# microsoft/UniSpeech

Hardware: AMD Instinct MI355X
Metric: audio-seconds/sec pretraining, WavLM-Base 15s@16kHz (higher is better)
Workload: dtype bf16; 1 GPU; WavLM-Base (12L, d=768) pretrain fwd+bwd+grad-reduce+fused-Adam, bf16, batch=32x15s per GPU, masked-pred loss (BASELINE.json configs[1]); global_batch=32, frames_per_utt=749, parallelism=dp1, optimizer=fused Adam, fp32 master, clip 10

## Files before the change

### include/wavlm_hip.h

```cpp
#ifndef WAVLM_HIP_H
#define WAVLM_HIP_H
#include <stddef.h>
#include <stdint.h>
#ifdef __cplusplus
extern "C" {
#endif

#define WAVLM_HIP_ABI_VERSION 29
int wavlm_abi_version(void);

typedef struct wavlm_gemm_desc {
  int32_t dtype;
  int32_t c_dtype;
  int32_t M, N, K, KB;
  int32_t transA, transB;
  int64_t lda, ldb, ldc;
  int64_t sA_kb, sB_kb;
  int32_t batch_o, batch_i;
  int64_t sA_o, sA_i, sB_o, sB_i, sC_o, sC_i;
  const void* A;
  const void* B;
  void* C;
  float alpha;
  int32_t epi;
// ... 208 lines not shown
  void* y;
  void* r_out;
  void* saved; uint64_t saved_bytes;
  void* workspace; uint64_t ws_bytes;
  const void* dy;
  const void* dr_out;
  void* dx;
  void* dr_in;
  float* dtab;
} wavlm_layer_desc;
uint64_t wavlm_layer_saved_bytes(const wavlm_layer_desc* d);
uint64_t wavlm_layer_fwd_workspace_bytes(const wavlm_layer_desc* d);
uint64_t wavlm_layer_bwd_workspace_bytes(const wavlm_layer_desc* d);
int wavlm_encoder_layer_fwd(const wavlm_layer_desc* d, void* stream);
int wavlm_encoder_layer_bwd(const wavlm_layer_desc* d, void* stream);

typedef void (*wavlm_grad_listener)(const void* base, uint64_t bytes, void* stream, void* user);
void wavlm_dp_set_listener(wavlm_grad_listener cb, void* user);

int wavlm_dp_unique_id(void* id128);
int wavlm_dp_init(int32_t rank, int32_t world, const void* id128, int32_t average);
int wavlm_dp_bucket_ready(void* base, uint64_t count, int32_t dtype, void* compute_stream);
int wavlm_dp_finish(void* compute_stream);
int wavlm_dp_destroy(void);

uint64_t wavlm_kmeans_centres_bytes(int32_t K, int32_t D);
int wavlm_kmeans_prepare(const float* C, int32_t K, int32_t D, void* image, uint64_t image_bytes, void* stream);
int wavlm_kmeans_assign(const void* X, int32_t x_dtype, int64_t N, int32_t D, int64_t ldx, const void* image, int32_t K,
                        int32_t* labels, float* min_dist, void* stream);
uint64_t wavlm_kmeans_accumulate_workspace_bytes(int64_t N, int32_t K, int32_t D);
// ... 72 lines not shown
```

### unispeech_amd/_lib.py

```python
import ctypes as C
import os

_HERE = os.path.dirname(os.path.abspath(__file__))
LIB_PATH = os.environ.get("WAVLM_HIP_LIB") or os.path.join(_HERE, "lib", "libwavlm_hip.so")

_lib = None
ABI_VERSION = 29

F32, BF16, I16 = 0, 1, 2

c_i32, c_i64, c_u64, c_f32, c_vp = C.c_int32, C.c_int64, C.c_uint64, C.c_float, C.c_void_p


class ConvRelayoutDesc(C.Structure):
    _fields_ = [("W", c_vp * 8), ("Wf", c_vp * 8), ("Wb", c_vp * 8),
                ("Cout", c_i32 * 8), ("Cin", c_i32 * 8), ("k", c_i32 * 8), ("s", c_i32 * 8),
                ("n_layers", c_i32), ("dtype", c_i32)]


class GemmDesc(C.Structure):
    _fields_ = [
        ("dtype", c_i32), ("c_dtype", c_i32),
        ("M", c_i32), ("N", c_i32), ("K", c_i32), ("KB", c_i32),
        ("transA", c_i32), ("transB", c_i32),
# ... 174 lines not shown
    "wavlm_mfcc_rows": (c_i32, [c_vp, c_i32, c_i64, c_i32, c_i64, c_vp, c_i32, c_i32, c_i32, c_vp, c_vp, c_vp, c_vp, c_i32, c_vp,
                                c_vp, c_i64, c_i64, c_i32, c_vp]),
    "wavlm_fbank_supported": (c_i32, [c_i32, c_i32, c_i32, c_i32]),
    "wavlm_fbank_frames": (c_i64, [c_i64, c_i32, c_i32]),
    "wavlm_fbank_rows": (c_i32, [c_vp, c_i32, c_i64, c_i32, c_i64, c_vp, c_i32, c_i32, c_i32, c_i32, c_vp, c_vp, c_vp, c_vp, c_i32,
                                 c_vp, c_i64, c_i64, c_vp]),
    "wavlm_dp_set_listener": (None, [c_vp, c_vp]),
    "wavlm_dp_unique_id": (c_i32, [c_vp]),
    "wavlm_dp_init": (c_i32, [c_i32, c_i32, c_vp, c_i32]),
    "wavlm_dp_bucket_ready": (c_i32, [c_vp, c_u64, c_i32, c_vp]),
    "wavlm_dp_finish": (c_i32, [c_vp]),
    "wavlm_dp_destroy": (c_i32, []),
    "wavlm_prof_enable": (None, [c_i32]),
    "wavlm_gemm_set_variant": (None, [c_i32]),
    "wavlm_set_reserved_cus": (None, [c_i32]),
    "wavlm_get_reserved_cus": (c_i32, []),
    "wavlm_prof_collect": (c_i32, [c_i32, C.POINTER(C.c_double), C.POINTER(C.c_double)]),
    "wavlm_prof_collect_bytes": (C.c_double, [c_i32]),
    "wavlm_prof_collect_class": (c_i32, [c_i32, C.POINTER(C.c_double), C.POINTER(C.c_double), C.POINTER(C.c_double)]),
    "wavlm_prof_dump": (c_i32, [C.c_char_p]),
}

_ERR = {-1: "invalid argument", -2: "kernel launch failure", -3: "out of memory"}


class WavlmHipError(RuntimeError):
    pass


def lib():
# ... 22 lines not shown
```

### unispeech_amd/csrc/attn_fused.hip

```cpp
#include "attn_fused.hpp"

typedef float f32x2_t __attribute__((ext_vector_type(2)));
#if !defined(WAVLM_EXPERIMENTAL)
#undef FA_FWD_LAZY
#undef FA_FWD_THETA
#undef FA_DQ_PK
#endif
#ifndef FA_FWD_LAZY
#define FA_FWD_LAZY 0
#endif
#ifndef FA_FWD_THETA
#define FA_FWD_THETA 8.f
#endif
#ifndef FA_DQ_PK
#define FA_DQ_PK 1
#endif
#if !defined(WAVLM_EXPERIMENTAL)
#undef FA_FWD_MFMA_SUM
#endif
#ifndef FA_FWD_MFMA_SUM
#define FA_FWD_MFMA_SUM 0
#endif
#ifndef FA_FWD_BIAS_IN_C
#define FA_FWD_BIAS_IN_C 1
// ... 780 lines not shown
    for (int f2 = 0; f2 < 2; ++f2)
#pragma unroll
      for (int q4 = 0; q4 < 4; ++q4) {
        uint2 w;
        w.x = pack_bf16(dq[f2][4 * q4] * p.scale, dq[f2][4 * q4 + 1] * p.scale);
        w.y = pack_bf16(dq[f2][4 * q4 + 2] * p.scale, dq[f2][4 * q4 + 3] * p.scale);
        *reinterpret_cast<uint2*>(dst + 32 * f2 + 8 * q4 + 4 * hi) = w;
      }
    if (hi == 0) {
      p.delta[(long)bh * T + i] = dl;
      if (p.dgate) p.dgate[(long)bh * T + i] = dg;
    }
  }
}

__global__ __launch_bounds__(1024) void fa_dtab_reduce_kernel(const float* __restrict__ part, float* __restrict__ out,
                                                              int B, int H, int nqt, int L, int Lp, int T, int nkv, int accumulate) {
  __shared__ float4 red[64][17];
  const int col = threadIdx.x & 15, slice = threadIdx.x >> 4;
  const int d = (blockIdx.x * 16 + col) * 4;
  const int h = blockIdx.y;
  const int nrow = nqt * 4, ntot = B * nrow, span = 64 * nkv + 32;
  float4 acc[4];
#pragma unroll
  for (int u = 0; u < 4; ++u) acc[u] = make_float4(0.f, 0.f, 0.f, 0.f);
  if (d < Lp) {
    for (int r0 = slice; r0 < ntot; r0 += 256) {
#pragma unroll
      for (int u = 0; u < 4; ++u) {
        const int r = r0 + 64 * u;
        if (r < ntot) {
          const int b = r / nrow, c = r - b * nrow;
          const int k0 = d - (T - 1 - 32 * c - 31);
          if (k0 > -4 && k0 < span) {
            const float4 v = *reinterpret_cast<const float4*>(part + (((long)b * H + h) * nrow + c) * Lp + d);
            acc[u].x += (k0 >= 0 && k0 < span) ? v.x : 0.f;
            acc[u].y += (k0 + 1 >= 0 && k0 + 1 < span) ? v.y : 0.f;
            acc[u].z += (k0 + 2 >= 0 && k0 + 2 < span) ? v.z : 0.f;
            acc[u].w += (k0 + 3 >= 0 && k0 + 3 < span) ? v.w : 0.f;
          }
        }
      }
    }
  }
  float4 t;
  t.x = (acc[0].x + acc[1].x) + (acc[2].x + acc[3].x); t.y = (acc[0].y + acc[1].y) + (acc[2].y + acc[3].y);
  t.z = (acc[0].z + acc[1].z) + (acc[2].z + acc[3].z); t.w = (acc[0].w + acc[1].w) + (acc[2].w + acc[3].w);
  red[slice][col] = t;
  __syncthreads();
  if (slice < 4) {
    float4 q = make_float4(0.f, 0.f, 0.f, 0.f);
#pragma unroll
    for (int k = 0; k < 16; ++k) { const float4 v = red[slice * 16 + k][col]; q.x += v.x; q.y += v.y; q.z += v.z; q.w += v.w; }
    red[slice * 16][col] = q;
  }
  __syncthreads();
  if (slice == 0 && d < L) {
    const float4 a0 = red[0][col], a1 = red[16][col], a2 = red[32][col], a3 = red[48][col];
    const float o[4] = {(a0.x + a1.x) + (a2.x + a3.x), (a0.y + a1.y) + (a2.y + a3.y), (a0.z + a1.z) + (a2.z + a3.z),
                        (a0.w + a1.w) + (a2.w + a3.w)};
#pragma unroll
    for (int k = 0; k < 4; ++k)
      if (d + k < L) out[(long)h * L + d + k] = accumulate ? out[(long)h * L + d + k] + o[k] : o[k];
  }
}

static FaP fa_params(int B, int H, int T, float scale, float p_drop, uint64_t seed) {
  FaP p;
  p.B = B; p.H = H; p.T = T; p.scale = scale;
  p.sc2 = scale * FA_LOG2E;
  double tt = (double)p_drop * 65536.0 + 0.5; if (tt > 65535.0) tt = 65535.0;
  p.th = p_drop > 0.f ? (unsigned)tt : 0u;
  if (p_drop > 0.f && p.th == 0u) p.th = 1u;
  p.sc = p.th ? (float)(1.0 / (1.0 - (double)p.th / 65536.0)) : 1.f;
  p.log2sc = log2f(p.sc); p.inv_sc = 1.f / p.sc;
  p.ths = (int)p.th - 32768;
  p.k2 = (unsigned)((p.ths - 1) & 0xffff) * 0x10001u;
  p.k3 = (unsigned)(p.ths & 0xffff) * 0x10001u;
  p.ps.P16 = nullptr; p.ps.mt = nullptr;
// ... 158 lines not shown
  if (use64) {
    p.nqb = (T + FA_K64 - 1) / FA_K64;
    const int rc = fa_launch_dkv64(p, (unsigned)(p.nqb * B * H), st);
    if (rc != WL_OK) return rc;
  } else {
    p.nqb = (T + FA_BK1 - 1) / FA_BK1;
    const dim3 grid2((unsigned)(p.nqb * B * H));
    const int rc = fa_launch_dkv(p, grid2.x, smem2, st);
    if (rc != WL_OK) return rc;
  }
  if (dbias) {
    const int rcb = wl_colsum_finish(p.dbias_part, B * nqt * 4, 3 * H * FA_HD, dbias, dbias_dtype, dbias_accumulate, st);
    if (rcb != WL_OK) return rcb;
    if (dbias_accumulate && !wl_fin_active()) wl_notify_grad(dbias, (uint64_t)3 * H * FA_HD * wl_esize(dbias_dtype), stream);
  }
  if (tab)
    WL_LAUNCH(fa_dtab_reduce_kernel, dim3((unsigned)((Lp / 4 + 15) / 16), (unsigned)H), dim3(1024), 0, st,
              (const float*)p.dtab_part, dtab, (int)B, (int)H, nqt, L, Lp, (int)T, (T + FA_BKV - 1) / FA_BKV, (int)dtab_accumulate);
  return wl_check_launch();
}
```

### unispeech_amd/csrc/common.hpp

```cpp
#pragma once
#include <hip/hip_runtime.h>
#include <stdint.h>
#include <stdio.h>
#include <mutex>

#define WL_MAX_DEVICES 64

#define WL_OK 0
#define WL_EINVAL (-1)
#define WL_ELAUNCH (-2)
#define WL_ENOMEM (-3)

enum { WL_F32 = 0, WL_BF16 = 1, WL_I16 = 2 };

typedef unsigned short bf16_t;

__device__ __forceinline__ float bf2f(bf16_t v) {
  return __uint_as_float(((unsigned)v) << 16);
}
__device__ __forceinline__ bf16_t f2bf(float f) {
  const __bf16 h = (__bf16)f;
  return __builtin_bit_cast(bf16_t, h);
}
__device__ __forceinline__ unsigned pack_bf16x2(float a, float b) {
// ... 157 lines not shown
  wl_launch_failed = 0;
  return e ? WL_ELAUNCH : WL_OK;
}

void wl_notify_grad(const void* base, uint64_t bytes, void* stream);
static inline uint64_t wl_esize(int dt) { return dt == WL_BF16 ? 2 : 4; }
int wl_attn_fused_bwd_ex(const void* qkv, const void* O, const void* dO, const float* lse, const float* gate,
                         const float* tab, const uint8_t* kpm, const void* pstore, uint64_t pstore_bytes, void* dqkv, float* dgate,
                         float* dtab, int dtab_accumulate,
                         void* dbias, int32_t dbias_dtype, int32_t dbias_accumulate, int32_t B, int32_t H, int32_t T,
                         int32_t head_dim, float scale, float p_drop, uint64_t seed, void* workspace, uint64_t ws_bytes,
                         void* stream);
int wl_colsum_finish(const float* part, int nblk, int n, void* out, int out_dtype, int accumulate, hipStream_t st);

struct WlFinSeg { const float* part; void* out; long stride, rep_stride; int nblk, n, out_dtype, accumulate, rep, blk0; };
#define WL_FIN_MAX 16
struct WlFinList { WlFinSeg s[WL_FIN_MAX]; int n, blocks; };
void wl_fin_defer(WlFinList* l);
bool wl_fin_active();
bool wl_fin_add(const float* part, int nblk, long stride, int n, void* out, int out_dtype, int accumulate, int rep = 1,
                long rep_stride = 0);
int wl_fin_flush(WlFinList& l, void* stream);
```

### unispeech_amd/csrc/gemm_bf16.hip

```cpp
#include <atomic>

#include "gemm_common.hpp"
#include "split_policy.hpp"

#include "tile_loaders.hpp"

template <bool TA, bool TB, int BM, int BN, int WM, int WN, bool VEC>
__global__ __launch_bounds__(WM * WN * 64) void gemm_bf16_kernel(GemmP p) {
  constexpr int FM = BM / WM / 32, FN = BN / WN / 32;
  constexpr int NT = WM * WN * 64;
  static_assert((WM * WN == 4 || WM * WN == 8) && FM >= 1 && FN >= 1, "4 or 8 waves");
  constexpr int A_BYTES = BM * 128, B_BYTES = BN * 128;
  extern __shared__ __attribute__((aligned(16))) unsigned char smem[];

  int tile;
  {
    const int nt = p.tiles_m * p.tiles_n, bid = blockIdx.x;
    const int q = nt >> 3, rem = nt & 7, xcd = bid & 7, idx = bid >> 3;
    tile = (xcd < rem ? xcd * (q + 1) : rem * (q + 1) + (xcd - rem) * q) + idx;
  }
  const int tn = tile % p.tiles_n, tm = tile / p.tiles_n;
  const int z = blockIdx.y, split = blockIdx.z;
  const int zo = z / p.batch_i, zi = z % p.batch_i;
  const int m0 = tm * BM, n0 = tn * BN;
// ... 151 lines not shown
      for (int u = 0; u < 4; ++u) {
        v[0] += a[u].x; v[1] += a[u].y; v[2] += a[u].z; v[3] += a[u].w;
        v[4] += b[u].x; v[5] += b[u].y; v[6] += b[u].z; v[7] += b[u].w;
      }
    }
    for (; k < S; ++k) {
      const float4 a = *reinterpret_cast<const float4*>(src + (long)k * mn);
      const float4 b = *reinterpret_cast<const float4*>(src + (long)k * mn + 4);
      v[0] += a.x; v[1] += a.y; v[2] += a.z; v[3] += a.w; v[4] += b.x; v[5] += b.y; v[6] += b.z; v[7] += b.w;
    }
    const int m = (int)(r / p.N), n = (int)(r - (long)m * p.N);
    gemm_store8(q, z / p.batch_i, z % p.batch_i, z, 0, m, n, v);
  }
}

struct RedGrpP {
  float* ws[4]; void* C[4]; long ldc[4]; int M[4], N[4], c_dtype[4], accumulate[4]; float alpha[4];
  long base[5]; int n, S;
};
__global__ __launch_bounds__(256) void gemm_splitk_reduce8_grouped_kernel(RedGrpP p) {
  const long total8 = p.base[p.n];
  for (long i8 = (long)blockIdx.x * blockDim.x + threadIdx.x; i8 < total8; i8 += (long)gridDim.x * blockDim.x) {
    const int g = (i8 >= p.base[1]) + (i8 >= p.base[2]) + (i8 >= p.base[3]);
    const long i = (i8 - p.base[g]) << 3;
    const int N = p.N[g];
    const long mn = (long)p.M[g] * N;
    const float* src = p.ws[g] + i;
    float v[8];
#pragma unroll
    for (int e = 0; e < 8; ++e) v[e] = 0.f;
    for (int k = 0; k < p.S; ++k) {
      const float4 a = *reinterpret_cast<const float4*>(src + (long)k * mn);
      const float4 b = *reinterpret_cast<const float4*>(src + (long)k * mn + 4);
      v[0] += a.x; v[1] += a.y; v[2] += a.z; v[3] += a.w; v[4] += b.x; v[5] += b.y; v[6] += b.z; v[7] += b.w;
    }
    const long m = i / N, n = i - m * N;
    const long off = m * p.ldc[g] + n;
#pragma unroll
    for (int e = 0; e < 8; ++e) v[e] *= p.alpha[g];
    if (p.accumulate[g]) {
      float c[8];
      ld8_dt(p.C[g], off, p.c_dtype[g], c);
#pragma unroll
      for (int e = 0; e < 8; ++e) v[e] += c[e];
    }
    st8_dt(p.C[g], off, p.c_dtype[g], v);
  }
}

template <bool TA, bool TB, int BM, int BN, int WM, int WN>
static int launch_cfg(GemmP& p, int nbatch, bool vec, hipStream_t st) {
  p.tiles_m = (p.M + BM - 1) / BM;
  p.tiles_n = (p.N + BN - 1) / BN;
  dim3 grid((unsigned)(p.tiles_m * p.tiles_n), (unsigned)nbatch, (unsigned)p.split_k);
  constexpr size_t smem = 2 * (size_t)(BM + BN) * 128;
  constexpr int nt = WM * WN * 64;
  if (smem > 65536) {
    static bool done_v = false, done_s = false;
    bool& done = vec ? done_v : done_s;
    if (!done) {
      const void* fn = vec ? (const void*)gemm_bf16_kernel<TA, TB, BM, BN, WM, WN, true>
                           : (const void*)gemm_bf16_kernel<TA, TB, BM, BN, WM, WN, false>;
// ... 355 lines not shown
    static const bool spread = [] { const char* e = getenv("WAVLM_SK_SPREAD"); return !(e && *e == '0'); }();
    p.sk_spread = spread && (plan.s * tiles_all) % 8 == 0 && plan.R % 8 == 0 && G % 8 == 0;
  }
  const int pi = prof_begin(d, st);
  if (pi >= 0) {
    g_prof.flops[pi] = flops;
    double by = 0.0;
    for (int i = 0; i < n; ++i) by += 2.0 * ((double)d[i].M * d[i].K + (double)d[i].N * d[i].K) + 2.0 * 2.0 * d[i].M * d[i].N;
    g_prof.bytes[pi] = by;
    int* sh = g_prof.shape[pi];
    sh[0] = -n; sh[1] = 0; sh[2] = d->K; sh[3] = 1; sh[4] = 3; sh[5] = 0; sh[6] = sk ? 0 : p.split_k; sh[7] = n;
  }
  const bool fixup = w4_takes(d, true) && gemm_w4_fixup_ok(p);
  p.fix_epoch = fixup ? 1u : 0u; p.fix_cnt = nullptr; p.fix_flag = nullptr;
  int rc = w4_takes(d, true) ? gemm_w4_launch_grouped(p, st) : gemm_pp_launch_grouped(p, st);
  if (rc == WL_OK && !fixup) {
    RedGrpP r;
    r.n = n; r.S = p.split_k; r.base[0] = 0;
    for (int i = 0; i < 4; ++i) {
      const wavlm_gemm_desc* e = d + (i < n ? i : n - 1);
      r.ws[i] = (float*)e->workspace; r.C[i] = e->C; r.ldc[i] = e->ldc; r.M[i] = e->M; r.N[i] = e->N;
      r.c_dtype[i] = e->c_dtype; r.accumulate[i] = e->accumulate; r.alpha[i] = e->alpha;
      r.base[i + 1] = i < n ? r.base[i] + (((long)e->M * e->N) >> 3) : 0x7fffffffffffffffL;
    }
    const long total8 = r.base[n];
    long blocks = (total8 + 255) / 256; if (blocks > 4096) blocks = 4096;
    WL_LAUNCH(gemm_splitk_reduce8_grouped_kernel, dim3((unsigned)blocks), dim3(256), 0, st, r);
    rc = wl_check_launch();
  }
  prof_end(pi, st);
  if (rc == WL_OK)
    for (int i = 0; i < n; ++i) gemm_notify(d + i, false, stream);
  return rc;
}
```

### unispeech_amd/csrc/layer.hip

```cpp
#include <stdlib.h>
#include <string.h>

#include <atomic>

#include "common.hpp"
#include "split_policy.hpp"
#include "wavlm_hip.h"

static std::atomic<wavlm_grad_listener> g_listener{nullptr};
static std::atomic<void*> g_listener_user{nullptr};
void wl_notify_grad(const void* base, uint64_t bytes, void* stream) {
  const wavlm_grad_listener cb = g_listener.load(std::memory_order_acquire);
  if (cb && base && bytes) cb(base, bytes, stream, g_listener_user.load(std::memory_order_acquire));
}
extern "C" void wavlm_dp_set_listener(wavlm_grad_listener cb, void* user) {
  g_listener.store(nullptr, std::memory_order_release);
  g_listener_user.store(user, std::memory_order_release);
  g_listener.store(cb, std::memory_order_release);
}

namespace {

inline uint64_t rup256(uint64_t v) { return (v + 255) & ~(uint64_t)255; }

// ... 114 lines not shown
  w.da = d->p_drop > 0.f ? c.take(n * D * 2) : w.dxa;
  w.dO = c.take(n * D * 2);
  w.dqkv = c.take(n * 3 * D * 2);
  if (d->tab) w.dgate = (float*)c.take((uint64_t)d->B * d->H * d->T * 4);
  w.ln_b = wavlm_layernorm_bwd_workspace_bytes(d->D); w.ln_ws = c.take(w.ln_b); w.ln_ws2 = c.take(w.ln_b);
  w.cs_b = lin_dx_colsum_ws((int64_t)n, d->F);
  if (w.cs_b < wavlm_colsum_workspace_bytes(d->D)) w.cs_b = wavlm_colsum_workspace_bytes(d->D);
  w.cs_ws = c.take(w.cs_b); w.cs_ws2 = c.take(w.cs_b);
  w.attn_b = wavlm_attn_fused_bwd_workspace_bytes(d->B, d->H, d->T); w.attn_ws = c.take(w.attn_b);
  w.gate_b = wavlm_gate_bwd_workspace_bytes(d->H, 64); w.gate_ws = c.take(w.gate_b);
  const wavlm_wgrad_item it[4] = {{nullptr, nullptr, nullptr, d->D, d->F}, {nullptr, nullptr, nullptr, d->F, d->D},
                                  {nullptr, nullptr, nullptr, d->D, d->D}, {nullptr, nullptr, nullptr, 3 * d->D, d->D}};
  w.wg_b = wavlm_linear_wgrads_workspace_bytes(it, 4, (int64_t)n); w.wg_ws = c.take(w.wg_b);
  w.bytes = c.off;
  if (base && !c.ok) w.bytes = ~(uint64_t)0;
  return w;
}

}

#if defined(WAVLM_EXPERIMENTAL)
extern "C" int wavlm_lab_build(void) { return 1; }
#endif

extern "C" {

static long grid_or(int32_t grid) { return grid > 0 ? grid : wl_policy::grid_blocks(); }
static int forced_or(int32_t forced) { return forced >= 0 ? forced : wl_policy::forced_split(); }
int32_t wavlm_grid_blocks(void) { return wl_policy::grid_blocks(); }
int32_t wavlm_wgrad_grouping(void) { return wl_policy::grouping() ? 1 : 0; }
// ... 15 lines not shown
    const long t = wg_tiles(it[i]);
    int s = wl_policy::split_single(it[i].N, it[i].K, kt, G);
    const int gs = wl_policy::slabs_grouped(t, kt, G, forced, false);
    if (gs > s) s = gs;
    if (balanced && t < G && G / t + 1 > s) s = (int)(G / t) + 1;
    tot += rup256((uint64_t)s * it[i].N * it[i].K * 4);
  }
  return tot;
}

int wavlm_linear_wgrads(const wavlm_wgrad_item* it, int32_t cnt, int64_t n, int32_t pdt, void* ws, uint64_t wsb, void* stream) {
  if (!it || cnt <= 0 || n <= 0 || (pdt != WL_BF16 && pdt != WL_F32)) return WL_EINVAL;
  for (int i = 0; i < cnt; ++i)
    if (!it[i].dy || !it[i].x || !it[i].dW || it[i].N <= 0 || it[i].K <= 0) return WL_EINVAL;
  const long kt = (long)((n + 63) / 64);
  int i = 0;
  while (i < cnt) {
    int j = i; long tiles = 0;
    while (wl_policy::grouping() && j < cnt && j - i < 4) {
      const long t = wg_tiles(it[j]);
      if (j > i && wavlm_split_grouped(tiles + t, kt, 0, -1) < 2) break;
      tiles += t; ++j;
    }
    if (j == i) j = i + 1;
    const int m = j - i;
    Carver c(ws, wsb);
    if (m >= 2) {
      const int split = wavlm_slabs_grouped(tiles, kt, 0, -1, -1);
      wavlm_gemm_desc g[4];
      for (int k = 0; k < m; ++k) {
        wg_desc(g[k], it[i + k], n, pdt, split);
        g[k].ws_bytes = wavlm_gemm_workspace_bytes(&g[k]);
        g[k].workspace = c.take(g[k].ws_bytes);
      }
      if (!c.ok) return WL_EINVAL;
      const int rc = wavlm_gemm_grouped(g, m, stream);
      if (rc != WL_OK) return rc;
    } else {
      wavlm_gemm_desc g;
      wg_desc(g, it[i], n, pdt, wavlm_split_single(it[i].N, it[i].K, kt, 0));
      if (g.split_k > 1) { g.ws_bytes = wavlm_gemm_workspace_bytes(&g); g.workspace = c.take(g.ws_bytes); if (!c.ok) return WL_EINVAL; }
// ... 139 lines not shown
```

### unispeech_amd/csrc/rowops.hip

```cpp
#include "common.hpp"
#include <stdlib.h>
#include "../../include/wavlm_hip.h"

__device__ __forceinline__ void load8(const float* p, float (&v)[8]) {
  const float4 a = *reinterpret_cast<const float4*>(p);
  const float4 b = *reinterpret_cast<const float4*>(p + 4);
  v[0] = a.x; v[1] = a.y; v[2] = a.z; v[3] = a.w; v[4] = b.x; v[5] = b.y; v[6] = b.z; v[7] = b.w;
}
__device__ __forceinline__ void load8(const bf16_t* p, float (&v)[8]) {
  const uint4 a = *reinterpret_cast<const uint4*>(p);
  v[0] = __uint_as_float(a.x << 16); v[1] = __uint_as_float(a.x & 0xffff0000u);
  v[2] = __uint_as_float(a.y << 16); v[3] = __uint_as_float(a.y & 0xffff0000u);
  v[4] = __uint_as_float(a.z << 16); v[5] = __uint_as_float(a.z & 0xffff0000u);
  v[6] = __uint_as_float(a.w << 16); v[7] = __uint_as_float(a.w & 0xffff0000u);
}
__device__ __forceinline__ void store8(float* p, const float (&v)[8]) {
  *reinterpret_cast<float4*>(p) = make_float4(v[0], v[1], v[2], v[3]);
  *reinterpret_cast<float4*>(p + 4) = make_float4(v[4], v[5], v[6], v[7]);
}
__device__ __forceinline__ void store8(bf16_t* p, const float (&v)[8]) {
  uint4 o;
  o.x = pack_bf16x2(v[0], v[1]); o.y = pack_bf16x2(v[2], v[3]);
  o.z = pack_bf16x2(v[4], v[5]); o.w = pack_bf16x2(v[6], v[7]);
  *reinterpret_cast<uint4*>(p) = o;
// ... 486 lines not shown
    }
    __syncthreads();
    for (int i = threadIdx.x; i < 64 * VEC; i += 256) {
      const int col = c * 64 * VEC + i;
      pg[col] = red[0][0][i] + red[1][0][i] + red[2][0][i] + red[3][0][i];
      pg[D + col] = red[0][1][i] + red[1][1][i] + red[2][1][i] + red[3][1][i];
      if constexpr (CS) pg[2 * D + col] = red[0][2][i] + red[1][2][i] + red[2][2][i] + red[3][2][i];
    }
  }
}

__global__ __launch_bounds__(1024) void colsum_finish_kernel(const float* __restrict__ part, int nblk, long stride, int n,
                                                              void* out, int out_dtype, int accumulate, long part_y, void* out_y,
                                                              void* out_z) {
  __shared__ float red[64][17];
  const int col = threadIdx.x & 15, slice = threadIdx.x >> 4;
  const int c = blockIdx.x * 16 + col;
  if (blockIdx.y) { part += part_y * blockIdx.y; out = blockIdx.y == 1 ? out_y : out_z; }
  float s = 0.f;
  if (c < n) {
    float s0 = 0.f, s1 = 0.f, s2 = 0.f, s3 = 0.f;
    int b = slice;
    for (; b + 192 < nblk; b += 256) {
      s0 += part[(long)b * stride + c];
      s1 += part[(long)(b + 64) * stride + c];
      s2 += part[(long)(b + 128) * stride + c];
      s3 += part[(long)(b + 192) * stride + c];
    }
    for (; b < nblk; b += 64) s0 += part[(long)b * stride + c];
    s = (s0 + s1) + (s2 + s3);
  }
  red[slice][col] = s;
  __syncthreads();
  if (slice < 4) {
    float t = 0.f;
#pragma unroll
    for (int k = 0; k < 16; ++k) t += red[slice * 16 + k][col];
    red[slice * 16][col] = t;
  }
  __syncthreads();
  if (slice == 0 && c < n) {
    s = (red[0][col] + red[16][col]) + (red[32][col] + red[48][col]);
    if (accumulate) s += ld_elem(out, c, out_dtype);
    st_elem(out, c, out_dtype, s);
  }
}

__global__ __launch_bounds__(1024) void colsum_finish_multi_kernel(WlFinList L) {
  __shared__ float red[64][17];
  int si = 0;
#pragma unroll 1
  for (int k = 1; k < L.n; ++k) if ((int)blockIdx.x >= L.s[k].blk0) si = k;
  const WlFinSeg& g = L.s[si];
  const float* __restrict__ part = g.part;
  const long stride = g.stride;
  const int nblk = g.nblk, n = g.n;
  const int col = threadIdx.x & 15, slice = threadIdx.x >> 4;
  const int c = ((int)blockIdx.x - g.blk0) * 16 + col;
  float s = 0.f;
  if (c < n) {
    float s0 = 0.f, s1 = 0.f, s2 = 0.f, s3 = 0.f;
    int b = slice;
    for (; b + 192 < nblk; b += 256) {
      s0 += part[(long)b * stride + c];
      s1 += part[(long)(b + 64) * stride + c];
      s2 += part[(long)(b + 128) * stride + c];
      s3 += part[(long)(b + 192) * stride + c];
    }
    for (; b < nblk; b += 64) s0 += part[(long)b * stride + c];
    s = (s0 + s1) + (s2 + s3);
  }
  red[slice][col] = s;
  __syncthreads();
  if (slice < 4) {
    float t = 0.f;
#pragma unroll
    for (int k = 0; k < 16; ++k) t += red[slice * 16 + k][col];
    red[slice * 16][col] = t;
  }
  __syncthreads();
  if (slice == 0 && c < n) {
    s = (red[0][col] + red[16][col]) + (red[32][col] + red[48][col]);
    for (int r = 0; r < g.rep; ++r) {
      const long idx = (long)r * g.rep_stride + c;
      st_elem(g.out, idx, g.out_dtype, g.accumulate ? s + ld_elem(g.out, idx, g.out_dtype) : s);
    }
  }
}

static thread_local WlFinList* g_fin_list = nullptr;
void wl_fin_defer(WlFinList* l) { g_fin_list = l; if (l) { l->n = 0; l->blocks = 0; } }
bool wl_fin_active() { return g_fin_list != nullptr; }
bool wl_fin_add(const float* part, int nblk, long stride, int n, void* out, int out_dtype, int accumulate, int rep, long rep_stride) {
  WlFinList* l = g_fin_list;
  if (!l || l->n >= WL_FIN_MAX || n <= 0) return false;
  WlFinSeg& g = l->s[l->n++];
  g.part = part; g.out = out; g.stride = stride; g.rep_stride = rep_stride; g.nblk = nblk; g.n = n; g.out_dtype = out_dtype;
  g.accumulate = accumulate; g.rep = rep < 1 ? 1 : rep; g.blk0 = l->blocks;
  l->blocks += (n + 15) / 16;
  return true;
}
int wl_fin_flush(WlFinList& l, void* stream) {
  if (l.n == 0) return WL_OK;
  WL_LAUNCH(colsum_finish_multi_kernel, dim3((unsigned)l.blocks), dim3(1024), 0, (hipStream_t)stream, l);
  const int rc = wl_check_launch();
  if (rc == WL_OK)
    for (int k = 0; k < l.n; ++k) {
      const WlFinSeg& g = l.s[k];
      if (g.accumulate) wl_notify_grad(g.out, (uint64_t)((long)(g.rep - 1) * g.rep_stride + g.n) * wl_esize(g.out_dtype), stream);
    }
  l.n = 0; l.blocks = 0;
  return rc;
}

#define CS_MAXC 8
template <typename T>
__global__ __launch_bounds__(256) void colsum_partial_kernel(const T* __restrict__ x, long rows, int N, long ld,
    const unsigned char* __restrict__ inc, const unsigned char* __restrict__ exc, float* __restrict__ part) {
  __shared__ float red[4][512];
  const int lane = threadIdx.x & 63, wave = threadIdx.x >> 6;
  const int nch = N >> 3;
  float acc[CS_MAXC][8];
#pragma unroll
  for (int c = 0; c < CS_MAXC; ++c)
#pragma unroll
    for (int e = 0; e < 8; ++e) acc[c][e] = 0.f;
// ... 531 lines not shown
```

Measured before the change: 14590 audio-s/s.

## Merge split-K slab, relative-bias and colsum finish reductions into one deferred kernel

Split-K grouped weight-gradient reductions and the attention relative-position-bias gradient reduction can now be deferred into the existing finish list and run in a single merged kernel alongside the bias column-sum finishes. The goal is fewer small kernel launches and less serialization at the end of each layer's backward pass. To make deferral safe, the weight-grad workspace carver stops reusing its buffer across groups while merging, and workspace overlap checks are added. This costs more workspace, delays gradient notifications until the flush, and uses a larger block size for the slab reduction.

```diff
diff --git a/include/wavlm_hip.h b/include/wavlm_hip.h
--- a/include/wavlm_hip.h
+++ b/include/wavlm_hip.h
@@ -6,7 +6,7 @@
 extern "C" {
 #endif
 
-#define WAVLM_HIP_ABI_VERSION 29
+#define WAVLM_HIP_ABI_VERSION 30
 int wavlm_abi_version(void);
 
 typedef struct wavlm_gemm_desc {
@@ -246,6 +246,8 @@
 uint64_t wavlm_layer_bwd_workspace_bytes(const wavlm_layer_desc* d);
 int wavlm_encoder_layer_fwd(const wavlm_layer_desc* d, void* stream);
 int wavlm_encoder_layer_bwd(const wavlm_layer_desc* d, void* stream);
+void wavlm_set_fin_merge(int on);
+int wavlm_get_fin_merge(void);
 
 typedef void (*wavlm_grad_listener)(const void* base, uint64_t bytes, void* stream, void* user);
 void wavlm_dp_set_listener(wavlm_grad_listener cb, void* user);
diff --git a/unispeech_amd/_lib.py b/unispeech_amd/_lib.py
--- a/unispeech_amd/_lib.py
+++ b/unispeech_amd/_lib.py
@@ -5,7 +5,7 @@
 LIB_PATH = os.environ.get("WAVLM_HIP_LIB") or os.path.join(_HERE, "lib", "libwavlm_hip.so")
 
 _lib = None
-ABI_VERSION = 29
+ABI_VERSION = 30
 
 F32, BF16, I16 = 0, 1, 2
 
@@ -212,6 +212,8 @@
     "wavlm_prof_enable": (None, [c_i32]),
     "wavlm_gemm_set_variant": (None, [c_i32]),
     "wavlm_set_reserved_cus": (None, [c_i32]),
+    "wavlm_set_fin_merge": (None, [c_i32]),
+    "wavlm_get_fin_merge": (c_i32, []),
     "wavlm_get_reserved_cus": (c_i32, []),
     "wavlm_prof_collect": (c_i32, [c_i32, C.POINTER(C.c_double), C.POINTER(C.c_double)]),
     "wavlm_prof_collect_bytes": (C.c_double, [c_i32]),
diff --git a/unispeech_amd/csrc/attn_fused.hip b/unispeech_amd/csrc/attn_fused.hip
--- a/unispeech_amd/csrc/attn_fused.hip
+++ b/unispeech_amd/csrc/attn_fused.hip
@@ -1,4 +1,5 @@
 #include "attn_fused.hpp"
+#include "fin_reduce.hpp"
 
 typedef float f32x2_t __attribute__((ext_vector_type(2)));
 #if !defined(WAVLM_EXPERIMENTAL)
@@ -818,55 +819,9 @@
   }
 }
 
-__global__ __launch_bounds__(1024) void fa_dtab_reduce_kernel(const float* __restrict__ part, float* __restrict__ out,
-                                                              int B, int H, int nqt, int L, int Lp, int T, int nkv, int accumulate) {
+__global__ __launch_bounds__(1024) void fa_dtab_reduce_kernel(WlDrelP p) {
   __shared__ float4 red[64][17];
-  const int col = threadIdx.x & 15, slice = threadIdx.x >> 4;
-  const int d = (blockIdx.x * 16 + col) * 4;
-  const int h = blockIdx.y;
-  const int nrow = nqt * 4, ntot = B * nrow, span = 64 * nkv + 32;
-  float4 acc[4];
-#pragma unroll
-  for (int u = 0; u < 4; ++u) acc[u] = make_float4(0.f, 0.f, 0.f, 0.f);
-  if (d < Lp) {
-    for (int r0 = slice; r0 < ntot; r0 += 256) {
-#pragma unroll
-      for (int u = 0; u < 4; ++u) {
-        const int r = r0 + 64 * u;
-        if (r < ntot) {
-          const int b = r / nrow, c = r - b * nrow;
-          const int k0 = d - (T - 1 - 32 * c - 31);
-          if (k0 > -4 && k0 < span) {
-            const float4 v = *reinterpret_cast<const float4*>(part + (((long)b * H + h) * nrow + c) * Lp + d);
-            acc[u].x += (k0 >= 0 && k0 < span) ? v.x : 0.f;
-            acc[u].y += (k0 + 1 >= 0 && k0 + 1 < span) ? v.y : 0.f;
-            acc[u].z += (k0 + 2 >= 0 && k0 + 2 < span) ? v.z : 0.f;
-            acc[u].w += (k0 + 3 >= 0 && k0 + 3 < span) ? v.w : 0.f;
-          }
-        }
-      }
-    }
-  }
-  float4 t;
-  t.x = (acc[0].x + acc[1].x) + (acc[2].x + acc[3].x); t.y = (acc[0].y + acc[1].y) + (acc[2].y + acc[3].y);
-  t.z = (acc[0].z + acc[1].z) + (acc[2].z + acc[3].z); t.w = (acc[0].w + acc[1].w) + (acc[2].w + acc[3].w);
-  red[slice][col] = t;
-  __syncthreads();
-  if (slice < 4) {
-    float4 q = make_float4(0.f, 0.f, 0.f, 0.f);
-#pragma unroll
-    for (int k = 0; k < 16; ++k) { const float4 v = red[slice * 16 + k][col]; q.x += v.x; q.y += v.y; q.z += v.z; q.w += v.w; }
-    red[slice * 16][col] = q;
-  }
-  __syncthreads();
-  if (slice == 0 && d < L) {
-    const float4 a0 = red[0][col], a1 = red[16][col], a2 = red[32][col], a3 = red[48][col];
-    const float o[4] = {(a0.x + a1.x) + (a2.x + a3.x), (a0.y + a1.y) + (a2.y + a3.y), (a0.z + a1.z) + (a2.z + a3.z),
-                        (a0.w + a1.w) + (a2.w + a3.w)};
-#pragma unroll
-    for (int k = 0; k < 4; ++k)
-      if (d + k < L) out[(long)h * L + d + k] = accumulate ? out[(long)h * L + d + k] + o[k] : o[k];
-  }
+  wl_drel_reduce_body(p, (int)blockIdx.x, (int)blockIdx.y, (int)threadIdx.x, red);
 }
 
 static FaP fa_params(int B, int H, int T, float scale, float p_drop, uint64_t seed) {
@@ -1055,8 +1010,10 @@
     if (rcb != WL_OK) return rcb;
     if (dbias_accumulate && !wl_fin_active()) wl_notify_grad(dbias, (uint64_t)3 * H * FA_HD * wl_esize(dbias_dtype), stream);
   }
-  if (tab)
-    WL_LAUNCH(fa_dtab_reduce_kernel, dim3((unsigned)((Lp / 4 + 15) / 16), (unsigned)H), dim3(1024), 0, st,
-              (const float*)p.dtab_part, dtab, (int)B, (int)H, nqt, L, Lp, (int)T, (T + FA_BKV - 1) / FA_BKV, (int)dtab_accumulate);
+  if (tab) {
+    const WlDrelP r = {(const float*)p.dtab_part, dtab, (int)B, (int)H, nqt, L, Lp, (int)T, (T + FA_BKV - 1) / FA_BKV, (int)dtab_accumulate};
+    if (!wl_fin_add_drel(r))
+      WL_LAUNCH(fa_dtab_reduce_kernel, dim3((unsigned)((Lp / 4 + 15) / 16), (unsigned)H), dim3(1024), 0, st, r);
+  }
   return wl_check_launch();
 }
diff --git a/unispeech_amd/csrc/common.hpp b/unispeech_amd/csrc/common.hpp
--- a/unispeech_amd/csrc/common.hpp
+++ b/unispeech_amd/csrc/common.hpp
@@ -195,10 +195,25 @@
 int wl_colsum_finish(const float* part, int nblk, int n, void* out, int out_dtype, int accumulate, hipStream_t st);
 
 struct WlFinSeg { const float* part; void* out; long stride, rep_stride; int nblk, n, out_dtype, accumulate, rep, blk0; };
+struct RedGrpP {
+  float* ws[4]; void* C[4]; long ldc[4]; int M[4], N[4], c_dtype[4], accumulate[4]; float alpha[4];
+  long base[5]; int n, S;
+};
+struct WlDrelP { const float* part; float* out; int B, H, nqt, L, Lp, T, nkv, accumulate; };
 #define WL_FIN_MAX 16
-struct WlFinList { WlFinSeg s[WL_FIN_MAX]; int n, blocks; };
+#define WL_FIN_SLAB_MAX 4
+#define WL_FIN_MERGE_DEFAULT 1
+#define WL_FIN_THREADS 1024
+struct WlFinList {
+  WlFinSeg s[WL_FIN_MAX]; RedGrpP slab[WL_FIN_SLAB_MAX]; WlDrelP drel;
+  int slab_blk0[WL_FIN_SLAB_MAX], slab_nblk[WL_FIN_SLAB_MAX];
+  int n, blocks, nslab, ndrel, drel_blk0, drel_gx, cs_blk0;
+};
 void wl_fin_defer(WlFinList* l);
 bool wl_fin_active();
 bool wl_fin_add(const float* part, int nblk, long stride, int n, void* out, int out_dtype, int accumulate, int rep = 1,
                 long rep_stride = 0);
+bool wl_fin_merging();
+bool wl_fin_add_slab(const RedGrpP& r);
+bool wl_fin_add_drel(const WlDrelP& r);
 int wl_fin_flush(WlFinList& l, void* stream);
diff --git a/unispeech_amd/csrc/fin_reduce.hpp b/unispeech_amd/csrc/fin_reduce.hpp
--- /dev/null
+++ b/unispeech_amd/csrc/fin_reduce.hpp
@@ -0,0 +1,119 @@
+#pragma once
+#include "gemm_common.hpp"
+
+__device__ __forceinline__ void wl_colsum_finish_body(const float* __restrict__ part, int nblk, long stride, int n, void* out,
+                                                      int out_dtype, int accumulate, int rep, long rep_stride, int blk, int tid,
+                                                      float (*red)[17]) {
+  const int col = tid & 15, slice = tid >> 4;
+  const int c = blk * 16 + col;
+  float s = 0.f;
+  if (c < n) {
+    float s0 = 0.f, s1 = 0.f, s2 = 0.f, s3 = 0.f;
+    int b = slice;
+    for (; b + 192 < nblk; b += 256) {
+      s0 += part[(long)b * stride + c];
+      s1 += part[(long)(b + 64) * stride + c];
+      s2 += part[(long)(b + 128) * stride + c];
+      s3 += part[(long)(b + 192) * stride + c];
+    }
+    for (; b < nblk; b += 64) s0 += part[(long)b * stride + c];
+    s = (s0 + s1) + (s2 + s3);
+  }
+  red[slice][col] = s;
+  __syncthreads();
+  if (slice < 4) {
+    float t = 0.f;
+#pragma unroll
+    for (int k = 0; k < 16; ++k) t += red[slice * 16 + k][col];
+    red[slice * 16][col] = t;
+  }
+  __syncthreads();
+  if (slice == 0 && c < n) {
+    s = (red[0][col] + red[16][col]) + (red[32][col] + red[48][col]);
+    for (int r = 0; r < rep; ++r) {
+      const long idx = (long)r * rep_stride + c;
+      st_elem(out, idx, out_dtype, accumulate ? s + ld_elem(out, idx, out_dtype) : s);
+    }
+  }
+}
+
+__device__ __forceinline__ void wl_slab_reduce_body(const RedGrpP& p, long first, long step) {
+  const long total8 = p.base[p.n];
+  for (long i8 = first; i8 < total8; i8 += step) {
+    const int g = (i8 >= p.base[1]) + (i8 >= p.base[2]) + (i8 >= p.base[3]);
+    const long i = (i8 - p.base[g]) << 3;
+    const int N = p.N[g];
+    const long mn = (long)p.M[g] * N;
+    const float* src = p.ws[g] + i;
+    float v[8];
+#pragma unroll
+    for (int e = 0; e < 8; ++e) v[e] = 0.f;
+    for (int k = 0; k < p.S; ++k) {
+      const float4 a = *reinterpret_cast<const float4*>(src + (long)k * mn);
+      const float4 b = *reinterpret_cast<const float4*>(src + (long)k * mn + 4);
+      v[0] += a.x; v[1] += a.y; v[2] += a.z; v[3] += a.w; v[4] += b.x; v[5] += b.y; v[6] += b.z; v[7] += b.w;
+    }
+    const long m = i / N, n = i - m * N;
+    const long off = m * p.ldc[g] + n;
+#pragma unroll
+    for (int e = 0; e < 8; ++e) v[e] *= p.alpha[g];
+    if (p.accumulate[g]) {
+      float c[8];
+      ld8_dt(p.C[g], off, p.c_dtype[g], c);
+#pragma unroll
+      for (int e = 0; e < 8; ++e) v[e] += c[e];
+    }
+    st8_dt(p.C[g], off, p.c_dtype[g], v);
+  }
+}
+
+__device__ __forceinline__ void wl_drel_reduce_body(const WlDrelP& p, int bx, int h, int tid, float4 (*red)[17]) {
+  const float* __restrict__ part = p.part;
+  float* __restrict__ out = p.out;
+  const int B = p.B, H = p.H, nqt = p.nqt, L = p.L, Lp = p.Lp, T = p.T, nkv = p.nkv, accumulate = p.accumulate;
+  const int col = tid & 15, slice = tid >> 4;
+  const int d = (bx * 16 + col) * 4;
+  const int nrow = nqt * 4, ntot = B * nrow, span = 64 * nkv + 32;
+  float4 acc[4];
+#pragma unroll
+  for (int u = 0; u < 4; ++u) acc[u] = make_float4(0.f, 0.f, 0.f, 0.f);
+  if (d < Lp) {
+    for (int r0 = slice; r0 < ntot; r0 += 256) {
+#pragma unroll
+      for (int u = 0; u < 4; ++u) {
+        const int r = r0 + 64 * u;
+        if (r < ntot) {
+          const int b = r / nrow, c = r - b * nrow;
+          const int k0 = d - (T - 1 - 32 * c - 31);
+          if (k0 > -4 && k0 < span) {
+            const float4 v = *reinterpret_cast<const float4*>(part + (((long)b * H + h) * nrow + c) * Lp + d);
+            acc[u].x += (k0 >= 0 && k0 < span) ? v.x : 0.f;
+            acc[u].y += (k0 + 1 >= 0 && k0 + 1 < span) ? v.y : 0.f;
+            acc[u].z += (k0 + 2 >= 0 && k0 + 2 < span) ? v.z : 0.f;
+            acc[u].w += (k0 + 3 >= 0 && k0 + 3 < span) ? v.w : 0.f;
+          }
+        }
+      }
+    }
+  }
+  float4 t;
+  t.x = (acc[0].x + acc[1].x) + (acc[2].x + acc[3].x); t.y = (acc[0].y + acc[1].y) + (acc[2].y + acc[3].y);
+  t.z = (acc[0].z + acc[1].z) + (acc[2].z + acc[3].z); t.w = (acc[0].w + acc[1].w) + (acc[2].w + acc[3].w);
+  red[slice][col] = t;
+  __syncthreads();
+  if (slice < 4) {
+    float4 q = make_float4(0.f, 0.f, 0.f, 0.f);
+#pragma unroll
+    for (int k = 0; k < 16; ++k) { const float4 v = red[slice * 16 + k][col]; q.x += v.x; q.y += v.y; q.z += v.z; q.w += v.w; }
+    red[slice * 16][col] = q;
+  }
+  __syncthreads();
+  if (slice == 0 && d < L) {
+    const float4 a0 = red[0][col], a1 = red[16][col], a2 = red[32][col], a3 = red[48][col];
+    const float o[4] = {(a0.x + a1.x) + (a2.x + a3.x), (a0.y + a1.y) + (a2.y + a3.y), (a0.z + a1.z) + (a2.z + a3.z),
+                        (a0.w + a1.w) + (a2.w + a3.w)};
+#pragma unroll
+    for (int k = 0; k < 4; ++k)
+      if (d + k < L) out[(long)h * L + d + k] = accumulate ? out[(long)h * L + d + k] + o[k] : o[k];
+  }
+}
diff --git a/unispeech_amd/csrc/gemm_bf16.hip b/unispeech_amd/csrc/gemm_bf16.hip
--- a/unispeech_amd/csrc/gemm_bf16.hip
+++ b/unispeech_amd/csrc/gemm_bf16.hip
@@ -1,6 +1,7 @@
 #include <atomic>
 
 #include "gemm_common.hpp"
+#include "fin_reduce.hpp"
 #include "split_policy.hpp"
 
 #include "tile_loaders.hpp"
@@ -189,38 +190,8 @@
   }
 }
 
-struct RedGrpP {
-  float* ws[4]; void* C[4]; long ldc[4]; int M[4], N[4], c_dtype[4], accumulate[4]; float alpha[4];
-  long base[5]; int n, S;
-};
 __global__ __launch_bounds__(256) void gemm_splitk_reduce8_grouped_kernel(RedGrpP p) {
-  const long total8 = p.base[p.n];
-  for (long i8 = (long)blockIdx.x * blockDim.x + threadIdx.x; i8 < total8; i8 += (long)gridDim.x * blockDim.x) {
-    const int g = (i8 >= p.base[1]) + (i8 >= p.base[2]) + (i8 >= p.base[3]);
-    const long i = (i8 - p.base[g]) << 3;
-    const int N = p.N[g];
-    const long mn = (long)p.M[g] * N;
-    const float* src = p.ws[g] + i;
-    float v[8];
-#pragma unroll
-    for (int e = 0; e < 8; ++e) v[e] = 0.f;
-    for (int k = 0; k < p.S; ++k) {
-      const float4 a = *reinterpret_cast<const float4*>(src + (long)k * mn);
-      const float4 b = *reinterpret_cast<const float4*>(src + (long)k * mn + 4);
-      v[0] += a.x; v[1] += a.y; v[2] += a.z; v[3] += a.w; v[4] += b.x; v[5] += b.y; v[6] += b.z; v[7] += b.w;
-    }
-    const long m = i / N, n = i - m * N;
-    const long off = m * p.ldc[g] + n;
-#pragma unroll
-    for (int e = 0; e < 8; ++e) v[e] *= p.alpha[g];
-    if (p.accumulate[g]) {
-      float c[8];
-      ld8_dt(p.C[g], off, p.c_dtype[g], c);
-#pragma unroll
-      for (int e = 0; e < 8; ++e) v[e] += c[e];
-    }
-    st8_dt(p.C[g], off, p.c_dtype[g], v);
-  }
+  wl_slab_reduce_body(p, (long)blockIdx.x * blockDim.x + threadIdx.x, (long)gridDim.x * blockDim.x);
 }
 
 template <bool TA, bool TB, int BM, int BN, int WM, int WN>
@@ -606,6 +577,7 @@
   const bool fixup = w4_takes(d, true) && gemm_w4_fixup_ok(p);
   p.fix_epoch = fixup ? 1u : 0u; p.fix_cnt = nullptr; p.fix_flag = nullptr;
   int rc = w4_takes(d, true) ? gemm_w4_launch_grouped(p, st) : gemm_pp_launch_grouped(p, st);
+  bool deferred = false;
   if (rc == WL_OK && !fixup) {
     RedGrpP r;
     r.n = n; r.S = p.split_k; r.base[0] = 0;
@@ -616,12 +588,15 @@
       r.base[i + 1] = i < n ? r.base[i] + (((long)e->M * e->N) >> 3) : 0x7fffffffffffffffL;
     }
     const long total8 = r.base[n];
-    long blocks = (total8 + 255) / 256; if (blocks > 4096) blocks = 4096;
-    WL_LAUNCH(gemm_splitk_reduce8_grouped_kernel, dim3((unsigned)blocks), dim3(256), 0, st, r);
-    rc = wl_check_launch();
+    deferred = wl_fin_add_slab(r);
+    if (!deferred) {
+      long blocks = (total8 + 255) / 256; if (blocks > 4096) blocks = 4096;
+      WL_LAUNCH(gemm_splitk_reduce8_grouped_kernel, dim3((unsigned)blocks), dim3(256), 0, st, r);
+      rc = wl_check_launch();
+    }
   }
   prof_end(pi, st);
-  if (rc == WL_OK)
+  if (rc == WL_OK && !deferred)
     for (int i = 0; i < n; ++i) gemm_notify(d + i, false, stream);
   return rc;
 }
diff --git a/unispeech_amd/csrc/layer.hip b/unispeech_amd/csrc/layer.hip
--- a/unispeech_amd/csrc/layer.hip
+++ b/unispeech_amd/csrc/layer.hip
@@ -152,6 +152,16 @@
   w.wg_b = wavlm_linear_wgrads_workspace_bytes(it, 4, (int64_t)n); w.wg_ws = c.take(w.wg_b);
   w.bytes = c.off;
   if (base && !c.ok) w.bytes = ~(uint64_t)0;
+  const struct { const void* p; uint64_t b; } piece[] = {
+      {w.dsa, n * D * 2}, {w.df, n * D * 2}, {w.du, n * F * 2}, {w.dh, n * D * 2}, {w.dxa, n * D * 2}, {w.da, n * D * 2},
+      {w.dO, n * D * 2}, {w.dqkv, n * 3 * D * 2}, {w.dgate, d->tab ? (uint64_t)d->B * d->H * d->T * 4 : 0}, {w.ln_ws, w.ln_b},
+      {w.ln_ws2, w.ln_b}, {w.cs_ws, w.cs_b}, {w.cs_ws2, w.cs_b}, {w.gate_ws, w.gate_b}, {w.attn_ws, w.attn_b}, {w.wg_ws, w.wg_b}};
+  const int np = (int)(sizeof(piece) / sizeof(piece[0]));
+  for (int k = np - 2; k < np; ++k)
+    for (int j = 0; j < np; ++j) {
+      const char *a0 = (const char*)piece[k].p, *b0 = (const char*)piece[j].p;
+      if (j != k && piece[j].b && piece[k].b && a0 < b0 + piece[j].b && b0 < a0 + piece[k].b) w.bytes = ~(uint64_t)0;
+    }
   return w;
 }
 
@@ -197,8 +207,11 @@
   for (int i = 0; i < cnt; ++i)
     if (!it[i].dy || !it[i].x || !it[i].dW || it[i].N <= 0 || it[i].K <= 0) return WL_EINVAL;
   const long kt = (long)((n + 63) / 64);
+  const bool keep = wl_fin_merging();
+  Carver c(ws, wsb);
   int i = 0;
   while (i < cnt) {
+    if (!keep) c = Carver(ws, wsb);
     int j = i; long tiles = 0;
     while (wl_policy::grouping() && j < cnt && j - i < 4) {
       const long t = wg_tiles(it[j]);
@@ -207,7 +220,6 @@
     }
     if (j == i) j = i + 1;
     const int m = j - i;
-    Carver c(ws, wsb);
     if (m >= 2) {
       const int split = wavlm_slabs_grouped(tiles, kt, 0, -1, -1);
       wavlm_gemm_desc g[4];
diff --git a/unispeech_amd/csrc/rowops.hip b/unispeech_amd/csrc/rowops.hip
--- a/unispeech_amd/csrc/rowops.hip
+++ b/unispeech_amd/csrc/rowops.hip
@@ -1,4 +1,4 @@
-#include "common.hpp"
+#include "fin_reduce.hpp"
 #include <stdlib.h>
 #include "../../include/wavlm_hip.h"
 
@@ -524,83 +524,47 @@
                                                               void* out, int out_dtype, int accumulate, long part_y, void* out_y,
                                                               void* out_z) {
   __shared__ float red[64][17];
-  const int col = threadIdx.x & 15, slice = threadIdx.x >> 4;
-  const int c = blockIdx.x * 16 + col;
   if (blockIdx.y) { part += part_y * blockIdx.y; out = blockIdx.y == 1 ? out_y : out_z; }
-  float s = 0.f;
-  if (c < n) {
-    float s0 = 0.f, s1 = 0.f, s2 = 0.f, s3 = 0.f;
-    int b = slice;
-    for (; b + 192 < nblk; b += 256) {
-      s0 += part[(long)b * stride + c];
-      s1 += part[(long)(b + 64) * stride + c];
-      s2 += part[(long)(b + 128) * stride + c];
-      s3 += part[(long)(b + 192) * stride + c];
-    }
-    for (; b < nblk; b += 64) s0 += part[(long)b * stride + c];
-    s = (s0 + s1) + (s2 + s3);
-  }
-  red[slice][col] = s;
-  __syncthreads();
-  if (slice < 4) {
-    float t = 0.f;
-#pragma unroll
-    for (int k = 0; k < 16; ++k) t += red[slice * 16 + k][col];
-    red[slice * 16][col] = t;
-  }
-  __syncthreads();
-  if (slice == 0 && c < n) {
-    s = (red[0][col] + red[16][col]) + (red[32][col] + red[48][col]);
-    if (accumulate) s += ld_elem(out, c, out_dtype);
-    st_elem(out, c, out_dtype, s);
-  }
-}
-
+  wl_colsum_finish_body(part, nblk, stride, n, out, out_dtype, accumulate, 1, 0, (int)blockIdx.x, (int)threadIdx.x, red);
+}
+
+__device__ __forceinline__ void fin_colsum_segment(const WlFinList& L, int blk, float (*red)[17]) {
+  int si = 0;
+#pragma unroll 1
+  for (int k = 1; k < L.n; ++k) if (blk >= L.s[k].blk0) si = k;
+  const WlFinSeg& g = L.s[si];
+  wl_colsum_finish_body(g.part, g.nblk, g.stride, g.n, g.out, g.out_dtype, g.accumulate, g.rep, g.rep_stride, blk - g.blk0,
+                        (int)threadIdx.x, red);
+}
 __global__ __launch_bounds__(1024) void colsum_finish_multi_kernel(WlFinList L) {
   __shared__ float red[64][17];
-  int si = 0;
+  fin_colsum_segment(L, (int)blockIdx.x, red);
+}
+
+__global__ __launch_bounds__(WL_FIN_THREADS) void fin_merged_kernel(WlFinList L) {
+  __shared__ float4 red4[64][17];
+  const int blk = (int)blockIdx.x;
+  if (blk >= L.cs_blk0) {
+    fin_colsum_segment(L, blk - L.cs_blk0, reinterpret_cast<float (*)[17]>(&red4[0][0]));
+  } else if (blk >= L.drel_blk0) {
+    const int lb = blk - L.drel_blk0, h = lb / L.drel_gx;
+    wl_drel_reduce_body(L.drel, lb - h * L.drel_gx, h, (int)threadIdx.x, red4);
+  } else {
+    int k = 0;
 #pragma unroll 1
-  for (int k = 1; k < L.n; ++k) if ((int)blockIdx.x >= L.s[k].blk0) si = k;
-  const WlFinSeg& g = L.s[si];
-  const float* __restrict__ part = g.part;
-  const long stride = g.stride;
-  const int nblk = g.nblk, n = g.n;
-  const int col = threadIdx.x & 15, slice = threadIdx.x >> 4;
-  const int c = ((int)blockIdx.x - g.blk0) * 16 + col;
-  float s = 0.f;
-  if (c < n) {
-    float s0 = 0.f, s1 = 0.f, s2 = 0.f, s3 = 0.f;
-    int b = slice;
-    for (; b + 192 < nblk; b += 256) {
-      s0 += part[(long)b * stride + c];
-      s1 += part[(long)(b + 64) * stride + c];
-      s2 += part[(long)(b + 128) * stride + c];
-      s3 += part[(long)(b + 192) * stride + c];
-    }
-    for (; b < nblk; b += 64) s0 += part[(long)b * stride + c];
-    s = (s0 + s1) + (s2 + s3);
-  }
-  red[slice][col] = s;
-  __syncthreads();
-  if (slice < 4) {
-    float t = 0.f;
-#pragma unroll
-    for (int k = 0; k < 16; ++k) t += red[slice * 16 + k][col];
-    red[slice * 16][col] = t;
-  }
-  __syncthreads();
-  if (slice == 0 && c < n) {
-    s = (red[0][col] + red[16][col]) + (red[32][col] + red[48][col]);
-    for (int r = 0; r < g.rep; ++r) {
-      const long idx = (long)r * g.rep_stride + c;
-      st_elem(g.out, idx, g.out_dtype, g.accumulate ? s + ld_elem(g.out, idx, g.out_dtype) : s);
-    }
-  }
-}
+    for (int q = 1; q < L.nslab; ++q) if (blk >= L.slab_blk0[q]) k = q;
+    wl_slab_reduce_body(L.slab[k], (long)(blk - L.slab_blk0[k]) * WL_FIN_THREADS + threadIdx.x, (long)L.slab_nblk[k] * WL_FIN_THREADS);
+  }
+}
+
+static int g_fin_merge = [] { const char* e = getenv("WAVLM_FIN_MERGE"); return e && *e ? (e[0] != '0' ? 1 : 0) : WL_FIN_MERGE_DEFAULT; }();
+extern "C" void wavlm_set_fin_merge(int on) { g_fin_merge = on ? 1 : 0; }
+extern "C" int wavlm_get_fin_merge(void) { return g_fin_merge; }
 
 static thread_local WlFinList* g_fin_list = nullptr;
-void wl_fin_defer(WlFinList* l) { g_fin_list = l; if (l) { l->n = 0; l->blocks = 0; } }
+void wl_fin_defer(WlFinList* l) { g_fin_list = l; if (l) { l->n = 0; l->blocks = 0; l->nslab = 0; l->ndrel = 0; } }
 bool wl_fin_active() { return g_fin_list != nullptr; }
+bool wl_fin_merging() { return g_fin_list != nullptr && g_fin_merge != 0; }
 bool wl_fin_add(const float* part, int nblk, long stride, int n, void* out, int out_dtype, int accumulate, int rep, long rep_stride) {
   WlFinList* l = g_fin_list;
   if (!l || l->n >= WL_FIN_MAX || n <= 0) return false;
@@ -610,16 +574,46 @@
   l->blocks += (n + 15) / 16;
   return true;
 }
+bool wl_fin_add_slab(const RedGrpP& r) {
+  WlFinList* l = g_fin_list;
+  if (!l || !g_fin_merge || l->nslab >= WL_FIN_SLAB_MAX || r.base[r.n] <= 0) return false;
+  l->slab[l->nslab++] = r;
+  return true;
+}
+bool wl_fin_add_drel(const WlDrelP& r) {
+  WlFinList* l = g_fin_list;
+  if (!l || !g_fin_merge || l->ndrel >= 1) return false;
+  l->drel = r; l->ndrel = 1;
+  return true;
+}
 int wl_fin_flush(WlFinList& l, void* stream) {
-  if (l.n == 0) return WL_OK;
-  WL_LAUNCH(colsum_finish_multi_kernel, dim3((unsigned)l.blocks), dim3(1024), 0, (hipStream_t)stream, l);
+  if (l.n == 0 && l.nslab == 0 && l.ndrel == 0) return WL_OK;
+  if (l.nslab == 0 && l.ndrel == 0) {
+    WL_LAUNCH(colsum_finish_multi_kernel, dim3((unsigned)l.blocks), dim3(1024), 0, (hipStream_t)stream, l);
+  } else {
+    int b = 0;
+    for (int k = 0; k < l.nslab; ++k) {
+      long nb = (l.slab[k].base[l.slab[k].n] + WL_FIN_THREADS - 1) / WL_FIN_THREADS; if (nb > 1024) nb = 1024;
+      l.slab_blk0[k] = b; l.slab_nblk[k] = (int)nb; b += (int)nb;
+    }
+    l.drel_blk0 = b; l.drel_gx = 1;
+    if (l.ndrel) { l.drel_gx = (l.drel.Lp / 4 + 15) / 16; b += l.drel_gx * l.drel.H; }
+    l.cs_blk0 = b;
+    WL_LAUNCH(fin_merged_kernel, dim3((unsigned)(b + l.blocks)), dim3(WL_FIN_THREADS), 0, (hipStream_t)stream, l);
+  }
   const int rc = wl_check_launch();
-  if (rc == WL_OK)
+  if (rc == WL_OK) {
+    for (int k = 0; k < l.nslab; ++k) {
+      const RedGrpP& r = l.slab[k];
+      for (int i = 0; i < r.n; ++i)
+        if (r.accumulate[i]) wl_notify_grad(r.C[i], ((uint64_t)(r.M[i] - 1) * r.ldc[i] + r.N[i]) * wl_esize(r.c_dtype[i]), stream);
+    }
     for (int k = 0; k < l.n; ++k) {
       const WlFinSeg& g = l.s[k];
       if (g.accumulate) wl_notify_grad(g.out, (uint64_t)((long)(g.rep - 1) * g.rep_stride + g.n) * wl_esize(g.out_dtype), stream);
     }
-  l.n = 0; l.blocks = 0;
+  }
+  l.n = 0; l.blocks = 0; l.nslab = 0; l.ndrel = 0;
   return rc;
 }
 
```

Result: no change. 14680 audio-s/s (median of 6 runs) (+0.6%).
